# df07/mcp-raytracer

Hardware: AMD Instinct MI355X
Metric: Msamples/sec (w×h×spp/s) Cornell 800×800 spp=256 @1/2/4/8 GPU (higher is better)
Workload: dtype f64

## Files before the change

### include/rt_amd.h

```cpp
#ifndef RT_AMD_H
#define RT_AMD_H

#include <stddef.h>
#include <stdint.h>

#ifdef __cplusplus
extern "C" {
#endif

#define RT_AMD_VERSION 3

enum {
    RT_OK = 0,
    RT_ERR_INVALID = 1,
    RT_ERR_DEVICE = 2,
    RT_ERR_RENDER = 3
};

enum { RT_PRECISION_REF = 0, RT_PRECISION_FP32 = 1 };
enum { RT_TRAVERSAL_FAST = 0, RT_TRAVERSAL_REFERENCE = 1, RT_TRAVERSAL_BRUTE = 2, RT_TRAVERSAL_AUTO = 3 };

typedef struct rt_camera rt_camera;

typedef struct {
// ... 63 lines not shown
                            uint64_t* work_counters);

int rt_camera_export(const rt_camera* cam, void* nodes, void* prims, void* materials, void* lights,
                     int32_t* prim_object);

int rt_debug_world_hit(rt_camera* cam, int32_t traversal, int32_t n, const float* orig, const float* dir,
                       double* out);

int rt_debug_math(int32_t n, const uint32_t* u, double* out);

int rt_debug_fp64(int32_t n, const double* x, double* out);

int rt_debug_pass_plan(int64_t units, int64_t unit_slots, int64_t chunks_per_slot, int64_t rec_bytes_per_unit,
                       int64_t budget_bytes, int64_t* pass_units);

int rt_debug_rng(uint32_t seed, uint32_t pixel, uint32_t sample, int32_t n, uint32_t* out);

int rt_device_count(int32_t* count);

int rt_camera_kernel_times(rt_camera* cam, float* path_ms, float* accum_ms);

#define RT_STATS_WORDS 8
int rt_camera_stats_words(rt_camera* cam, uint64_t* dst, void* stream);

int rt_camera_adaptive_info(rt_camera* cam, int32_t* rounds, uint64_t* samples_rendered);

int rt_camera_pass_count(rt_camera* cam, int32_t* passes);

enum { RT_KERNEL_NONE = 0, RT_KERNEL_SEQUENTIAL = 1, RT_KERNEL_CHUNKED = 2, RT_KERNEL_POOL = 3 };
int rt_camera_last_kernel(rt_camera* cam, int32_t* kernel);
// ... 104 lines not shown
```

### mcp-raytracer_amd/csrc/rt_api.cpp

```cpp
#include <hip/hip_runtime.h>

#include <dlfcn.h>
#include <rccl/rccl.h>

#include <algorithm>
#include <cmath>
#include <cstddef>
#include <cstdio>
#include <cstdlib>
#include <cstring>
#include <exception>
#include <functional>
#include <memory>
#include <mutex>
#include <stdexcept>
#include <string>
#include <thread>
#include <type_traits>
#include <vector>

#include "../../include/rt_amd.h"
#include "denoise.hpp"
#include "json.hpp"
#include "launch.hpp"
#include "progressive.hpp"
#include "scene.hpp"

using namespace rt;

std::vector<uint8_t> rt_png_encode_device(const uint8_t* d_rgb, int32_t w, int32_t h, hipStream_t stream);

static_assert(ST_WORDS == RT_STATS_WORDS, "rt_camera_stats_words layout");

#ifndef RT_BUILD_ID
#define RT_BUILD_ID "unhashed"
#endif

namespace {

// ... 210 lines not shown
    DevCtx(const CamHost& h, int dev, int inst) : host(h), build(h.build), device(dev), instance(inst) {}
    DevCtx(const DevCtx&) = delete;
    DevCtx& operator=(const DevCtx&) = delete;

    uint4* d_blob = nullptr;
    int32_t lds_words = 0;
    int32_t lds_words2 = 0;
    int32_t off_prims = 0, off_mats = 0, off_lights = 0, off_nodes = 0, off_tprims = 0, off_tsph = 0, off_onbs = 0;
    int32_t off_tsph2 = -1;
    int32_t off_pre = 0, n_pre = 0, off_xrec = 0;
    int32_t n_onb = 0;
    int lds_max = 64 * 1024;
    std::vector<hipEvent_t> ev;
    int n_passes = 0;
    bool ev_accum = false;
    int last_kernel = RT_KERNEL_NONE;
    unsigned long long* d_stats = nullptr;
    unsigned long long* d_counters = nullptr;
    unsigned int* d_tile = nullptr;
    uint8_t* d_rgb = nullptr;
    float* d_rad = nullptr;
    int cus = 256;

    hipStream_t stream = nullptr;
    hipEvent_t ev_rendered = nullptr, ev_gather0 = nullptr, ev_gather1 = nullptr;
    uint8_t* d_slab = nullptr;
    float* d_rslab = nullptr;
    uint8_t* d_gather = nullptr;
    float* d_rgather = nullptr;
    size_t slab_cap = 0, rslab_cap = 0, gather_cap = 0, rgather_cap = 0;
    unsigned long long* h_words = nullptr;
    int h_words_cap = 0;

    ~DevCtx() {
// ... 32 lines not shown
        if (h_words_cap < n) {
            if (h_words) (void)hipHostFree(h_words);
            h_words = nullptr;
            h_words_cap = 0;
            hip_check(hipHostMalloc((void**)&h_words, (size_t)n * ST_WORDS * sizeof(unsigned long long), 0),
                      "hipHostMalloc");
            h_words_cap = n;
        }
    }

    void release() {
        if (!live) return;
        int prev = 0;
        (void)hipGetDevice(&prev);
        (void)hipSetDevice(device);
        for (void* p : {(void*)d_blob, (void*)d_stats, (void*)d_counters, (void*)d_tile, (void*)d_rgb, (void*)d_rad,
                        (void*)d_sbuf})
            if (p) (void)hipFree(p);
        d_blob = nullptr;
        d_stats = nullptr;
        d_counters = nullptr;
        d_tile = nullptr;
        d_rgb = nullptr;
        d_rad = nullptr;
        d_sbuf = nullptr;
        sbuf_cap = 0;
        free_adapt_buffers();
        prog_free();
        dn.free();
        if (d_prim_object) (void)hipFree(d_prim_object);
        d_prim_object = nullptr;
        for (hipEvent_t& e : dn_ev)
            if (e) (void)hipEventDestroy(e), e = nullptr;
// ... 143 lines not shown
        append(blob, build.tsph, &off_tsph);
        append(blob, build.prims, &off_prims);
        append(blob, exact_records(build.prims), &off_xrec);
        lds_words = (int32_t)(blob.size() / 16);
        append(blob, build.mats, &off_mats);
        append(blob, build.lights, &off_lights);
        const std::vector<RtOnb> onbs = planar_onbs(build.prims, &n_onb);
        append(blob, onbs, &off_onbs);
        lds_words2 = (int32_t)(blob.size() / 16);
        append(blob, build.nodes, &off_nodes);
        append(blob, prefilter_records(build.prims, &n_pre), &off_pre);
        off_tsph2 = -1;
        if (!build.tsph2.empty()) append(blob, build.tsph2, &off_tsph2);
        hip_check(hipMalloc(&d_blob, std::max<size_t>(blob.size(), 16)), "hipMalloc");
        if (!blob.empty()) hip_check(hipMemcpy(d_blob, blob.data(), blob.size(), hipMemcpyHostToDevice), "hipMemcpy");
        hip_check(hipMalloc(&d_stats, ST_WORDS * kStatStride * sizeof(unsigned long long)), "hipMalloc");
        hip_check(hipMalloc(&d_counters, kCounterWords * sizeof(unsigned long long)), "hipMalloc");
        hip_check(hipMalloc(&d_tile, 64), "hipMalloc");
        live = true;
        cus = device_cus(dev);
        int smem = 0;
        if (hipDeviceGetAttribute(&smem, hipDeviceAttributeMaxSharedMemoryPerBlock, dev) == hipSuccess && smem > 0)
            lds_max = smem;
    }

    void ensure_frame() {
        if (d_rgb) return;
        const size_t px = (size_t)build.cam.width * build.cam.height;
        hip_check(hipMalloc(&d_rgb, std::max<size_t>(px * 3, 1)), "hipMalloc");
        hip_check(hipMalloc(&d_rad, std::max<size_t>(px * 3, 1) * sizeof(float)), "hipMalloc");
    }

    hipEvent_t pass_event(int p, int k) {
        while ((int)ev.size() < 3 * (p + 1)) {
            hipEvent_t e = nullptr;
            hip_check(hipEventCreate(&e), "hipEventCreate");
            ev.push_back(e);
        }
        return ev[3 * p + k];
    }

    int effective_traversal(int trav) const { return host.effective_traversal(trav); }

    void times(float* path_ms, float* accum_ms) {
        *path_ms = 0.0f;
        *accum_ms = 0.0f;
        for (int p = 0; p < n_passes; ++p) {
            float a = 0.0f, b = 0.0f;
            hip_check(hipEventSynchronize(ev[3 * p + 1]), "hipEventSynchronize");
            hip_check(hipEventElapsedTime(&a, ev[3 * p], ev[3 * p + 1]), "hipEventElapsedTime");
            *path_ms += a;
            if (ev_accum) {
                hip_check(hipEventSynchronize(ev[3 * p + 2]), "hipEventSynchronize");
                hip_check(hipEventElapsedTime(&b, ev[3 * p + 1], ev[3 * p + 2]), "hipEventElapsedTime");
                *accum_ms += b;
            }
        }
    }

    DevScene dev_scene() const {
        DevScene S;
        const char* b = reinterpret_cast<const char*>(d_blob);
        S.tnodes = reinterpret_cast<const RtTNode*>(b);
        S.prims = reinterpret_cast<const RtPrim*>(b + off_prims);
        S.gprims = S.prims;
        S.gpre = reinterpret_cast<const RtPre*>(b + off_pre);
        S.n_pre = n_pre;
        S.xrec = reinterpret_cast<const RtExact*>(b + off_xrec);
        S.off_xrec = off_xrec;
// ... 20 lines not shown
        S.t4_stride = (int32_t)sizeof(RtT4Node);
        S.n_top = 0;
        S.top_lds = nullptr;
        S.nearfar = 0;
        S.troot = build.t4root;
        S.root_box = build.troot_box;
        S.cam = build.cam;
        S.mix_total = host.mix_total;
        S.light_w = host.light_w;
        return S;
    }

    void launch(const rt_region& region, int tile_group, int tile_groups, int prec, int trav, int count,
                uint8_t* rgb, float* rad, int32_t* pxs, int32_t* pxb, int packed, hipStream_t stream,
                int prog_len = 0) {
        const RtCamera& C = build.cam;
        if (tile_groups < 1 || tile_group < 0 || tile_group >= tile_groups)
            throw std::invalid_argument("tile_group must satisfy 0 <= tile_group < tile_groups");
        const int x0 = std::max(region.x, 0), y0 = std::max(region.y, 0);
        const int x1 = std::min(region.x + region.width, C.width);
        const int y1 = std::min(region.y + region.height, C.height);
        RtRegion reg{x0, y0, std::max(x1 - x0, 0), std::max(y1 - y0, 0), tile_group, tile_groups};
        const int tiles_x = (reg.width + kTile - 1) / kTile;
        const int tiles_y = (reg.height + kTile - 1) / kTile;
        const long total = (long)tiles_x * tiles_y;
        const long mine = total > tile_group ? (total - tile_group + tile_groups - 1) / tile_groups : 0;
        LaunchGeom g;
        g.tiles_x = std::max(tiles_x, 1);
        g.my_tiles = (int)mine;
        const long want = (mine + (kBlock / kWave) - 1) / (kBlock / kWave);
// ... 21 lines not shown
        if (g.lds_level == 0 && v.trav == TRAV_FAST && lds_scene_enabled() && env_flag("RT_AMD_TOP_CACHE", true)) {
            const size_t room = lds_cap > stack ? lds_cap - stack : 0;
            n_top = (int32_t)std::min<size_t>(build.t4nodes.size(), room / node_lds);
            g.lds_bytes = stack + (size_t)n_top * node_lds;
        }
        v.defer = v.trav == TRAV_FAST &&
                  env_flag("RT_AMD_DEFER", g.lds_level >= 1 && C.n_prims >= 100);
        if (g.lds_bytes + static_lds_bytes(count, false) > (size_t)lds_max)
            throw std::runtime_error("traversal stack exceeds the workgroup LDS (BVH too deep)");
        if (env_flag("RT_AMD_LAUNCH_LOG", false))
            std::fprintf(stderr,
                         "[rt launch] prims %d stack_depth %d trav %d lds_level %d lds %zu B (stack %zu, scene L1 %d / "
                         "L2 %d B) lds_max %d tiles %ld\n",
                         C.n_prims, C.stack_depth, v.trav, g.lds_level, g.lds_bytes, stack, lds_words * 16,
                         lds_words2 * 16, lds_max, mine);
        RenderOut out{rgb, rad, pxs, pxb, d_stats, d_counters, d_tile, packed ? 1 : 0};
        hip_check(launch_init_stats(d_stats, count ? d_counters : nullptr, d_tile, stream), "init_stats");
        n_passes = 0;
        last_kernel = RT_KERNEL_NONE;
        adapt_rounds = 0;
        adapt_rendered = 0;
        if (mine == 0) return;
        DevScene S = dev_scene();
        S.lds_stack_bytes = (int32_t)stack;
        S.lds_words = g.lds_level == 2 ? lds_words2 : lds_words;
        S.lds_node_pad = g.lds_level > 0 ? node_pad : 0;
        S.n_top = n_top;
        S.tsph2 = off_tsph2 >= 0 ? reinterpret_cast<const RtLeafSph*>(reinterpret_cast<const char*>(d_blob) + off_tsph2)
                                 : nullptr;
        if (g.lds_level == 0 && v.trav == TRAV_FAST && !S.tsph2 && C.n_prims > 0)
            throw std::runtime_error("fast traversal without leaf records");
        const bool chunked = env_flag("RT_AMD_CHUNKED", true);
        const bool rounds = C.adaptive && count != 1 && env_flag("RT_AMD_ADAPT_ROUNDS", true);
        if (prog_len <= 0 && (C.n_samples <= 0 || !chunked || (C.adaptive && !rounds))) {
            hip_check(hipEventRecord(pass_event(0, 0), stream), "hipEventRecord");
            hipError_t e = prec == PREC_FP32 ? launch_render_fp32(v, S, reg, out, g, nullptr, stream)
                                             : launch_render_ref(v, S, reg, out, g, nullptr, stream);
            hip_check(e, "pt_render_kernel launch");
            hip_check(hipEventRecord(pass_event(0, 1), stream), "hipEventRecord");
            n_passes = 1;
            ev_accum = false;
            last_kernel = RT_KERNEL_SEQUENTIAL;
            return;
        }
        SampleBuf sb{};

        S.lds_pool_off = (int32_t)((g.lds_bytes + 15) / 16 * 16);
        const bool pool_ok = !v.emit && (count == 0 || (RT_POOL_PROF && count == 2 && prec == PREC_REF)) && v.trav == TRAV_BRUTE && C.width < 65536 && C.height < 65536 &&
                 C.n_samples <= 65535 && C.depth <= 250 && build.mats.size() < (1u << 21) &&
// ... 46 lines not shown
            if (covered != nsamp) throw std::runtime_error("guided schedule: coverage");
            for (int p = 0; p < np; ++p) sb.rnch[p] = 1.0 / (double)sb.nch[p];
            sb.refill_min = std::min(env_int("RT_AMD_REFILL", 4), kWave);
            sb.min_ready = std::min(env_int("RT_AMD_READY", gtree ? 40 : 48), kWave);
        };
        int pass = 0;
        auto run_pass = [&](bool first) {
            const long group_slots = ((long)sb.slots + kWave - 1) / kWave * kWave;
            long items = 0;
            for (int p = 0; p < sb.n_phases; ++p) {
                sb.item_base[p] = (int32_t)items;
                items += group_slots * sb.nch[p];
            }
            if (items >= kItemCap) throw std::runtime_error("chunked pass too large");
            sb.n_items = (int32_t)items;
            if (!first) hip_check(hipMemsetAsync(d_tile, 0, 2 * sizeof(unsigned int), stream), "hipMemsetAsync");
            LaunchGeom gp = g;
            const int block = v.pool ? kBlockPool : kBlockChunk;
            gp.grid = (int)std::max<long>(1, std::min<long>(items / block + 1, (long)cus));
            DevScene Sp = S;
            if (v.pool) gp.lds_bytes = (size_t)S.lds_pool_off + pool_lds_bytes();
            hip_check(hipEventRecord(pass_event(pass, 0), stream), "hipEventRecord");
            hipError_t e = prec == PREC_FP32 ? launch_render_fp32(v, Sp, reg, out, gp, &sb, stream)
                                             : launch_render_ref(v, Sp, reg, out, gp, &sb, stream);
            hip_check(e, "pt_chunk_kernel launch");
            hip_check(hipEventRecord(pass_event(pass, 1), stream), "hipEventRecord");
        };
        if (prog_len > 0) {
            launch_progressive(S, reg, out, g, sb, schedule, run_pass, pass, stream, prog_len);
        } else if (rounds) {
            launch_adaptive_rounds(S, reg, out, g, mine, sb, schedule, run_pass, pass, stream);
        } else {
            sb.rec12 = C.mode != MODE_BOUNCES && !out.px_bounces && env_flag("RT_AMD_REC12", true);
            const size_t rec_per_tile = (size_t)kWave * (size_t)C.n_samples * (sb.rec12 ? 12 : sizeof(float4));
            schedule((double)mine * kWave, C.n_samples);
            const long pass_tiles = pass_units(mine, kWave, chunks_per_slot(sb), rec_per_tile, sbuf_budget());
            ensure_sbuf((size_t)pass_tiles * rec_per_tile);
            sb.rec = d_sbuf;
            for (long t0 = 0; t0 < mine; t0 += pass_tiles, ++pass) {
                const long nt = std::min(pass_tiles, mine - t0);
                sb.tile0 = (int32_t)t0;
                sb.slots = (int32_t)(nt * kWave);
                if (env_flag("RT_AMD_REC_SLOT_MAJOR", false)) {
                    sb.stride_s = 1;
                    sb.stride_slot = C.n_samples;
                } else {
                    sb.stride_s = sb.slots;
                    sb.stride_slot = 1;
                }
                run_pass(t0 == 0);
                hip_check(launch_accum(S, reg, out, g.tiles_x, sb, stream), "pt_accum_kernel launch");
                hip_check(hipEventRecord(pass_event(pass, 2), stream), "hipEventRecord");
            }
        }
        n_passes = pass;
        ev_accum = true;
        last_kernel = v.pool ? RT_KERNEL_POOL : RT_KERNEL_CHUNKED;
    }

    template <class Sched, class Pass>
    void launch_adaptive_rounds(DevScene& S, const RtRegion& reg, const RenderOut& out, const LaunchGeom& g, long mine,
                                SampleBuf& sb, Sched& schedule, Pass& run_pass, int& pass, hipStream_t stream) {
        const RtCamera& C = build.cam;
        const long slots_all = mine * kWave;
        ensure_adapt((size_t)slots_all);
        const double ab = C.a_batch;
        const int batch = (ab >= 1.0 && ab < 65536.0) ? (int)ab : std::max(1, std::min(C.n_samples, 16));
        int len = batch * std::max(1, (env_int("RT_AMD_ADAPT_FIRST", batch) + batch - 1) / batch);
// ... 138 lines not shown

    void prog_read(hipStream_t stream) {
        ProgSession& P = prog;
        unsigned long long wl[ST_WORDS * kStatStride];
        hip_check(hipMemcpyAsync(wl, d_stats, sizeof wl, hipMemcpyDeviceToHost, stream), "hipMemcpyAsync");
        hip_check(hipMemcpyAsync(P.h_count, P.d_count, 2 * sizeof(unsigned int), hipMemcpyDeviceToHost, stream),
                  "hipMemcpyAsync");
        hip_check(hipStreamSynchronize(stream), "hipStreamSynchronize");
        for (int k = 0; k < ST_WORDS; ++k) P.words[k] = wl[k * kStatStride];
        P.err |= P.words[ST_ERROR];
        P.words[ST_ERROR] = P.err;
        P.n_act = (long)P.h_count[0];
    }

    void prog_start(hipStream_t stream) {
        hip_check(launch_init_stats(d_stats, nullptr, d_tile, stream), "init_stats");
        prog_resolve(stream);
        prog_read(stream);
    }

    template <class Sched, class Pass>
    void launch_progressive(DevScene& S, const RtRegion& reg, const RenderOut& out, const LaunchGeom& g, SampleBuf& sb,
                            Sched& schedule, Pass& run_pass, int& pass, hipStream_t stream, int len) {
        ProgSession& P = prog;
        const long n_act = P.n_act;
        sb.s_base = P.done;
        sb.err_in_rec = 1;
        sb.rec12 = 0;
        sb.stride_slot = 1;
        sb.tile0 = 0;
        schedule((double)n_act, len);
        const size_t rec_per_slot = (size_t)len * sizeof(float4);
        const long pass_slots =
// ... 58 lines not shown
        free_adapt_buffers();
        hip_check(hipMalloc(&d_astate, slots * sizeof(AdaptPix)), "hipMalloc(adaptive state)");
        hip_check(hipMalloc(&d_act[0], slots * sizeof(int32_t)), "hipMalloc(active list)");
        hip_check(hipMalloc(&d_act[1], slots * sizeof(int32_t)), "hipMalloc(active list)");
        adapt_cap = slots;
    }
    void free_adapt_buffers() {
        for (void* p : {(void*)d_astate, (void*)d_act[0], (void*)d_act[1]})
            if (p) (void)hipFree(p);
        d_astate = nullptr;
        d_act[0] = d_act[1] = nullptr;
        adapt_cap = 0;
    }

    float4* d_sbuf = nullptr;
    size_t sbuf_cap = 0;
    void ensure_sbuf(size_t bytes) {
        if (bytes <= sbuf_cap) return;
        if (d_sbuf) (void)hipFree(d_sbuf);
        d_sbuf = nullptr;
        sbuf_cap = 0;
        hip_check(hipMalloc(&d_sbuf, bytes), "hipMalloc(sample buffer)");
        sbuf_cap = bytes;
    }
    static long chunks_per_slot(const SampleBuf& sb) {
        long n = 0;
        for (int p = 0; p < sb.n_phases; ++p) n += sb.nch[p];
        return n;
    }
    static size_t sbuf_budget() {
        const char* e = std::getenv("RT_AMD_SBUF_MB");
        const long mb = e ? std::atol(e) : 8192;
        return (size_t)std::max<long>(mb, 1) << 20;
    }

    void read_stats(rt_render_stats* st, uint64_t* counters, hipStream_t stream) {
        unsigned long long wl[ST_WORDS * kStatStride], w[ST_WORDS];
        hip_check(hipMemcpyAsync(wl, d_stats, sizeof wl, hipMemcpyDeviceToHost, stream), "hipMemcpyAsync");
// ... 199 lines not shown

    std::vector<std::exception_ptr> errs(n);
    auto work = [&](int g) {
        try {
            DevCtx& c = *cs[g];
            hip_check(hipSetDevice(c.device), "hipSetDevice");
            c.ensure_device();
            c.ensure_multi(slab_b, rslab_b, g == 0, n);
            if (g == 0) c.ensure_frame();
            c.launch(plan.region, g, n, cam->precision, cam->traversal, 0, c.d_slab, want_rad ? c.d_rslab : nullptr,
                     nullptr, nullptr, 1, c.stream);
            hip_check(hipMemcpy2DAsync(c.d_slab + plan.stats_offset, sizeof(unsigned long long), c.d_stats,
                                       kStatStride * sizeof(unsigned long long), sizeof(unsigned long long), ST_WORDS,
                                       hipMemcpyDeviceToDevice, c.stream),
                      "hipMemcpy2DAsync(stats)");
            hip_check(hipEventRecord(c.ev_rendered, c.stream), "hipEventRecord");
        } catch (...) {
            errs[g] = std::current_exception();
        }
    };
    std::vector<std::thread> th;
    for (int g = 1; g < n; ++g) th.emplace_back(work, g);
    work(0);
    for (auto& t : th) t.join();
    for (auto& e : errs)
        if (e) std::rethrow_exception(e);

    DevCtx& root = *cs[0];
    hip_check(hipSetDevice(root.device), "hipSetDevice");
    hip_check(hipEventRecord(root.ev_gather0, root.stream), "hipEventRecord");
// ... 518 lines not shown
        if (d_out) (void)hipFree(d_out);
        return set_error(RT_ERR_DEVICE, e.what());
    }
}

int rt_debug_pass_plan(int64_t units, int64_t unit_slots, int64_t chunks_per_slot, int64_t rec_bytes_per_unit,
                       int64_t budget_bytes, int64_t* pass_units_out) {
    if (units < 0 || unit_slots < 1 || chunks_per_slot < 1 || rec_bytes_per_unit < 1 || budget_bytes < 1 ||
        !pass_units_out)
        return set_error(RT_ERR_INVALID, "bad arguments");
    *pass_units_out = pass_units((long)units, (long)unit_slots, (long)chunks_per_slot, (size_t)rec_bytes_per_unit,
                                 (size_t)budget_bytes);
    return RT_OK;
}

int rt_debug_rng(uint32_t seed, uint32_t pixel, uint32_t sample, int32_t n, uint32_t* out) {
    if (n < 0 || (n > 0 && !out)) return set_error(RT_ERR_INVALID, "bad arguments");
    uint64_t s = splitmix64((((uint64_t)pixel << 32) | sample) ^ splitmix64(seed));
    for (int32_t k = 0; k < n; ++k) {
        const uint64_t old = s;
        s = old * 6364136223846793005ull + 1442695040888963407ull;
        const uint32_t xs = (uint32_t)(((old >> 18u) ^ old) >> 27u);
        const uint32_t rot = (uint32_t)(old >> 59u);
        out[k] = (xs >> rot) | (xs << ((32u - rot) & 31u));
    }
    return RT_OK;
}

int rt_camera_kernel_times(rt_camera* cam, float* path_ms, float* accum_ms) {
    if (!cam || !path_ms || !accum_ms) return set_error(RT_ERR_INVALID, "null argument");
// ... 5 lines not shown
        return RT_OK;
    } catch (const std::exception& e) {
        return set_error(RT_ERR_DEVICE, e.what());
    }
}

int rt_camera_stats_words(rt_camera* cam, uint64_t* dst, void* stream) {
    if (!cam || !dst) return set_error(RT_ERR_INVALID, "null argument");
    std::lock_guard<std::mutex> lock(cam->mu);
    try {
        DevCtx* c = cam->last;
        if (!c || !c->live || !c->d_stats) throw std::invalid_argument("rt_camera_stats_words: no render yet");
        hip_check(hipMemcpy2DAsync(dst, sizeof(uint64_t), c->d_stats, kStatStride * sizeof(unsigned long long),
                                   sizeof(uint64_t), ST_WORDS, hipMemcpyDeviceToDevice, (hipStream_t)stream),
                  "hipMemcpy2DAsync(stats)");
        return RT_OK;
    } catch (const std::invalid_argument& e) {
        return set_error(RT_ERR_INVALID, e.what());
    } catch (const std::exception& e) {
        return set_error(RT_ERR_DEVICE, e.what());
    }
}

int rt_camera_adaptive_info(rt_camera* cam, int32_t* rounds, uint64_t* samples_rendered) {
    if (!cam || !rounds || !samples_rendered) return set_error(RT_ERR_INVALID, "null argument");
    std::lock_guard<std::mutex> lock(cam->mu);
    *rounds = cam->last ? cam->last->adapt_rounds : 0;
    *samples_rendered = cam->last ? cam->last->adapt_rendered : 0;
    return RT_OK;
}
// ... 527 lines not shown
```

### mcp-raytracer_amd/raytracer_amd/_build.py

```python
from __future__ import annotations

import hashlib
import os
import shutil
import subprocess
from concurrent.futures import ThreadPoolExecutor
from pathlib import Path

PKG_DIR = Path(__file__).resolve().parent
CSRC = PKG_DIR.parent / "csrc"
INCLUDE = PKG_DIR.parent.parent / "include"
LIB_DIR = PKG_DIR / "lib"
LIB_PATH = LIB_DIR / "librt_amd.so"
OBJ_DIR = PKG_DIR.parent / "build"

ARCH = "gfx950"

_COMMON = ["-std=c++17", "-O3", "-fPIC", "-Wall", "-Wno-unused-function", "-Wno-unused-variable",
           f"-I{CSRC}", f"-I{INCLUDE}"]

_KERNEL_FLAGS = ["-fno-slp-vectorize", "-mllvm", "-disable-machine-licm"]
_UNITS = [
    ("pt_ref.hip", ["-ffp-contract=off", *_KERNEL_FLAGS], True),
    ("pt_fp32.hip", ["-ffp-contract=fast", *_KERNEL_FLAGS], True),
    ("progressive.hip", ["-ffp-contract=off", *_KERNEL_FLAGS], True),
    ("denoise.hip", ["-ffp-contract=off", *_KERNEL_FLAGS], True),
    ("frame.hip", [], True),
    ("png.hip", [], True),
    ("rt_api.cpp", ["-ffp-contract=off", "-x", "hip"], True),
    ("scene.cpp", ["-ffp-contract=off"], False),
    ("image.cpp", [], False),
]
_HEADERS = ["json.hpp", "rt_math.hpp", "scene.hpp", "pt_kernel.hpp", "launch.hpp", "progressive.hpp", "denoise.hpp",
            "png_deflate.hpp"]
_LIBS = ["-lz"]


def source_hash(defines=(), flags=()) -> str:
    h = hashlib.sha256()
    for name in [u[0] for u in _UNITS] + _HEADERS:
        h.update(name.encode() + b"\0" + (CSRC / name).read_bytes())
    h.update((INCLUDE / "rt_amd.h").read_bytes())
    h.update(repr((ARCH, _COMMON[:3], [(u[0], u[1]) for u in _UNITS], _LIBS, list(defines), list(flags))).encode())
    return h.hexdigest()[:16]


def id_path(lib_path: Path) -> Path:
    return lib_path.with_name(lib_path.name + ".id")

# ... 76 lines not shown
```

### mcp-raytracer_amd/raytracer_amd/_lib.py

```python
from __future__ import annotations

import ctypes as C
import json
import os
from pathlib import Path

from ._build import LIB_PATH, id_path, source_hash

HEADER = Path(__file__).resolve().parents[2] / "include" / "rt_amd.h"

RT_OK, RT_ERR_INVALID, RT_ERR_DEVICE, RT_ERR_RENDER = 0, 1, 2, 3
PRECISION = {"ref": 0, "fp32": 1}
TRAVERSAL = {"fast": 0, "reference": 1, "brute": 2, "auto": 3}

CT_NAMES = ["node", "sphere", "quad", "plane", "material", "light_quad", "light_sphere",
            "bounces", "diffuse", "samples", "rays", "exact", "exact_wave", "cand0", "cand2", "exact2"]
PR_NAMES = ["newpath", "rr", "hit", "miss", "hitrec", "scatter", "sample", "pdf", "acc", "tile", "node", "leaf",
            "wnode", "wleaf", "loop", "trips"]
COUNTER_WORDS = 64
STATS_WORDS = 8


class RtRegion(C.Structure):
    _fields_ = [("x", C.c_int32), ("y", C.c_int32), ("width", C.c_int32), ("height", C.c_int32)]
# ... 54 lines not shown
                "samples_done": self.samples_done, "samples": self.samples, "steps": self.steps,
                "done": bool(self.done), "precision": "fp32" if self.precision == 1 else "ref", "seed": self.seed,
                "active_pixels": self.active_pixels, "state_bytes": self.state_bytes,
                "build_id": self.build_id.decode()}


class RtDenoiseOptions(C.Structure):
    _fields_ = [("levels", C.c_int32), ("sigma_color", C.c_float), ("sigma_plane", C.c_float)]


class RtDenoiseVarOptions(C.Structure):
    _fields_ = [("levels", C.c_int32), ("sigma_variance", C.c_float), ("sigma_plane", C.c_float)]


DENOISE_MAX_LEVELS = 8


class RtError(RuntimeError):

    def __init__(self, code: int, message: str):
        super().__init__(message)
        self.code = code


_SIGS = {
    "rt_version": (C.c_int, []),
    "rt_last_error": (C.c_char_p, []),
    "rt_free": (None, [C.c_void_p]),
    "rt_generate_scene_data": (C.c_int, [C.c_char_p, C.c_char_p, C.POINTER(C.c_void_p)]),
    "rt_camera_create": (C.c_int, [C.c_char_p, C.c_char_p, C.POINTER(C.c_void_p)]),
    "rt_camera_destroy": (None, [C.c_void_p]),
    "rt_camera_get_info": (C.c_int, [C.c_void_p, C.POINTER(RtCameraInfo)]),
    "rt_camera_set_precision": (C.c_int, [C.c_void_p, C.c_int32]),
    "rt_camera_render_region": (C.c_int, [C.c_void_p, C.POINTER(RtRegion), C.c_void_p, C.c_void_p,
                                          C.POINTER(RtRenderStats)]),
    "rt_camera_render": (C.c_int, [C.c_void_p, C.c_void_p, C.c_void_p, C.POINTER(RtRenderStats)]),
    "rt_camera_render_device": (C.c_int, [C.c_void_p, C.POINTER(RtLaunch), C.POINTER(RtRenderStats),
                                          C.POINTER(C.c_uint64)]),
    "rt_camera_export": (C.c_int, [C.c_void_p, C.c_void_p, C.c_void_p, C.c_void_p, C.c_void_p,
                                   C.c_void_p]),
    "rt_debug_world_hit": (C.c_int, [C.c_void_p, C.c_int32, C.c_int32, C.c_void_p, C.c_void_p, C.c_void_p]),
    "rt_debug_pass_plan": (C.c_int, [C.c_int64, C.c_int64, C.c_int64, C.c_int64, C.c_int64,
                                     C.POINTER(C.c_int64)]),
    "rt_debug_rng": (C.c_int, [C.c_uint32, C.c_uint32, C.c_uint32, C.c_int32, C.c_void_p]),
    "rt_debug_math": (C.c_int, [C.c_int32, C.c_void_p, C.c_void_p]),
    "rt_debug_fp64": (C.c_int, [C.c_int32, C.c_void_p, C.c_void_p]),
    "rt_device_count": (C.c_int, [C.POINTER(C.c_int32)]),
    "rt_camera_kernel_times": (C.c_int, [C.c_void_p, C.POINTER(C.c_float), C.POINTER(C.c_float)]),
    "rt_camera_adaptive_info": (C.c_int, [C.c_void_p, C.POINTER(C.c_int32), C.POINTER(C.c_uint64)]),
    "rt_camera_stats_words": (C.c_int, [C.c_void_p, C.c_void_p, C.c_void_p]),
    "rt_camera_pass_count": (C.c_int, [C.c_void_p, C.POINTER(C.c_int32)]),
    "rt_camera_last_kernel": (C.c_int, [C.c_void_p, C.POINTER(C.c_int32)]),
    "rt_camera_release_device": (C.c_int, [C.c_void_p]),
    "rt_build_id": (C.c_char_p, []),
    "rt_tiles_unpack": (C.c_int, [C.c_void_p, C.c_int32, C.c_int32, C.POINTER(RtRegion), C.c_int32, C.c_int32,
                                  C.c_int32, C.c_int32, C.c_void_p, C.c_void_p]),
    "rt_encode_png": (C.c_int, [C.c_void_p, C.c_int32, C.c_int32, C.c_int32, C.POINTER(C.c_void_p),
                                C.POINTER(C.c_size_t)]),
# ... 85 lines not shown

def to_json(obj) -> bytes:
    return json.dumps(obj, allow_nan=True, separators=(",", ":")).encode()


def multi_plan(region, width: int, height: int, n_devices: int) -> dict:
    p = RtMultiPlan()
    reg = RtRegion(*[int(v) for v in region])
    check(load().rt_multi_plan_region(C.byref(reg), int(width), int(height), int(n_devices), C.byref(p)))
    return {"region": (p.region.x, p.region.y, p.region.width, p.region.height), "n_devices": p.n_devices,
            "slab_tiles": p.slab_tiles, "tiles": p.tiles, "slab_bytes_rgb": p.slab_bytes_rgb,
            "slab_bytes_radiance": p.slab_bytes_radiance, "stats_offset": p.stats_offset,
            "group_tiles": list(p.group_tiles)[:p.n_devices]}


def progressive_blob_info(blob: bytes) -> dict:
    info = RtProgressiveInfo()
    blob = bytes(blob)
    check(load().rt_progressive_blob_info(blob, len(blob), C.byref(info)))
    return info.as_dict()


def progressive_blob_variance(blob: bytes):
    import numpy as np
    blob = bytes(blob)
    info = progressive_blob_info(blob)
    var = np.zeros((info["height"], info["width"]), np.float32)
    check(load().rt_progressive_blob_variance(blob, len(blob), var.ctypes.data))
    return var

# ... 6 lines not shown
```

### mcp-raytracer_amd/raytracer_amd/camera.py

```python
from __future__ import annotations

import ctypes as C
import math
from dataclasses import dataclass, field
from typing import Iterable, Optional, Sequence

from . import _lib

RENDER_MODES = ("default", "bounces", "samples")


def _mm(total=0.0, mn=math.inf, mx=0.0, avg=0.0):
    return {"total": total, "min": mn, "max": mx, "avg": avg}


@dataclass
class RenderStats:

    pixels: float = 0
    samples: dict = field(default_factory=_mm)
    bounces: dict = field(default_factory=_mm)

    @classmethod
    def _from_c(cls, s: _lib.RtRenderStats) -> "RenderStats":
# ... 258 lines not shown
        return float(a.value), float(b.value)

    def stats_words(self, dst_ptr: int, stream=None) -> None:
        _lib.check(self._lib.rt_camera_stats_words(self._h, C.c_void_p(dst_ptr), C.c_void_p(stream)))

    def adaptive_info(self):
        r, n = C.c_int32(), C.c_uint64()
        _lib.check(self._lib.rt_camera_adaptive_info(self._h, C.byref(r), C.byref(n)))
        return int(r.value), int(n.value)

    def pass_count(self) -> int:
        n = C.c_int32()
        _lib.check(self._lib.rt_camera_pass_count(self._h, C.byref(n)))
        return int(n.value)

    KERNELS = ("none", "sequential", "chunked", "pool")

    def last_kernel(self) -> str:
        n = C.c_int32()
        _lib.check(self._lib.rt_camera_last_kernel(self._h, C.byref(n)))
        return self.KERNELS[int(n.value)]

    def progressive(self, region=None) -> "ProgressiveRender":
        reg = None if region is None else _region(region)
        _lib.check(self._lib.rt_camera_progressive_begin(self._h, C.byref(reg) if reg is not None else None))
        return ProgressiveRender(self)

    def resume(self, blob: bytes) -> "ProgressiveRender":
        blob = bytes(blob)
        _lib.check(self._lib.rt_camera_progressive_restore(self._h, blob, len(blob)))
# ... 204 lines not shown
```

Before: 12120.

## Pipeline path-trace and accumulation passes with double-buffered sample records

Adds a second sample-record buffer and a second stats/counter/tile block, and runs the chunked path-tracing kernel on a separate non-blocking stream. The accumulation kernel stays on the caller stream and the two are ordered through a small event plan, so pass N's accumulate can overlap pass N+1's path kernel and a new launch can start while the previous one's accumulate is still running. This targets serialisation between passes and between back-to-back launches. In exchange it costs extra device memory for the second record buffer, adds event bookkeeping on every launch, and risks ordering bugs around stats reads, which is why block_read hooks are added.

```diff
diff --git a/include/rt_amd.h b/include/rt_amd.h
--- a/include/rt_amd.h
+++ b/include/rt_amd.h
@@ -101,6 +101,31 @@
 int rt_debug_pass_plan(int64_t units, int64_t unit_slots, int64_t chunks_per_slot, int64_t rec_bytes_per_unit,
                        int64_t budget_bytes, int64_t* pass_units);
 
+enum {
+    RT_PIPE_PATH0 = 1, RT_PIPE_PATH1 = 2, RT_PIPE_ACC0 = 4, RT_PIPE_ACC1 = 8, RT_PIPE_BLK0 = 16, RT_PIPE_BLK1 = 32
+};
+typedef struct {
+    int32_t have_second;
+    int32_t last_buf;
+    int32_t last_blk;
+    int32_t recorded;
+    int32_t tail;
+} rt_pipe_state;
+typedef struct {
+    int32_t pipelined;
+    int32_t buf, blk;
+    int32_t init_block;
+    int32_t alloc_second;
+    int32_t internal_waits;
+    int32_t internal_records;
+    int32_t caller_waits;
+    int32_t caller_records;
+} rt_pipe_pass;
+int rt_debug_pipeline_plan(rt_pipe_state* state, int32_t pipelined, int32_t passes, int32_t first_buffer_idle,
+                           rt_pipe_pass* out);
+
+int rt_camera_record_bytes(rt_camera* cam, int64_t* first, int64_t* second);
+
 int rt_debug_rng(uint32_t seed, uint32_t pixel, uint32_t sample, int32_t n, uint32_t* out);
 
 int rt_device_count(int32_t* count);
diff --git a/mcp-raytracer_amd/csrc/pipeline.hpp b/mcp-raytracer_amd/csrc/pipeline.hpp
--- /dev/null
+++ b/mcp-raytracer_amd/csrc/pipeline.hpp
@@ -0,0 +1,60 @@
+#pragma once
+
+#include <cstdint>
+
+#include "../../include/rt_amd.h"
+
+namespace rt {
+
+constexpr int32_t pipe_path_bit(int buf) { return buf ? RT_PIPE_PATH1 : RT_PIPE_PATH0; }
+constexpr int32_t pipe_acc_bit(int buf) { return buf ? RT_PIPE_ACC1 : RT_PIPE_ACC0; }
+constexpr int32_t pipe_blk_bit(int blk) { return blk ? RT_PIPE_BLK1 : RT_PIPE_BLK0; }
+constexpr int kPipeEvents = 6;
+
+inline rt_pipe_pass pipe_plan_pass(rt_pipe_state& s, bool pipelined, bool first, bool buf0_idle) {
+    rt_pipe_pass p{};
+    p.pipelined = pipelined ? 1 : 0;
+    p.init_block = first ? 1 : 0;
+    if (!pipelined) {
+        p.buf = 0;
+        p.blk = s.last_blk;
+        if (first) {
+            p.caller_waits = s.tail;
+            s.tail = 0;
+        }
+        s.last_buf = 0;
+        return p;
+    }
+    p.blk = first && (s.recorded & (RT_PIPE_BLK0 | RT_PIPE_BLK1)) ? 1 - s.last_blk : s.last_blk;
+    if (s.have_second) {
+        p.buf = 1 - s.last_buf;
+    } else if ((s.recorded & RT_PIPE_ACC0) && !(first && buf0_idle)) {
+        p.buf = 1;
+        p.alloc_second = 1;
+        s.have_second = 1;
+    } else {
+        p.buf = 0;
+    }
+    p.internal_waits = s.recorded & (pipe_acc_bit(p.buf) | (first ? pipe_blk_bit(p.blk) : 0));
+    p.internal_records = pipe_path_bit(p.buf);
+    p.caller_waits = pipe_path_bit(p.buf);
+    p.caller_records = pipe_acc_bit(p.buf);
+    s.recorded |= p.internal_records | p.caller_records;
+    s.tail = pipe_path_bit(p.buf);
+    s.last_buf = p.buf;
+    s.last_blk = p.blk;
+    return p;
+}
+
+inline int32_t pipe_plan_end(rt_pipe_state& s, bool pipelined) {
+    const int32_t r = pipe_blk_bit(s.last_blk) | (pipelined ? 0 : RT_PIPE_ACC0);
+    s.recorded |= r;
+    return r;
+}
+
+inline void pipe_plan_launch(rt_pipe_state& s, bool pipelined, int passes, bool buf0_idle, rt_pipe_pass* out) {
+    for (int p = 0; p < passes; ++p) out[p] = pipe_plan_pass(s, pipelined, p == 0, p == 0 && buf0_idle);
+    out[passes - 1].caller_records |= pipe_plan_end(s, pipelined);
+}
+
+}
diff --git a/mcp-raytracer_amd/csrc/rt_api.cpp b/mcp-raytracer_amd/csrc/rt_api.cpp
--- a/mcp-raytracer_amd/csrc/rt_api.cpp
+++ b/mcp-raytracer_amd/csrc/rt_api.cpp
@@ -23,6 +23,7 @@
 #include "denoise.hpp"
 #include "json.hpp"
 #include "launch.hpp"
+#include "pipeline.hpp"
 #include "progressive.hpp"
 #include "scene.hpp"
 
@@ -263,10 +264,18 @@
     std::vector<hipEvent_t> ev;
     int n_passes = 0;
     bool ev_accum = false;
+    bool ev_split = false;
     int last_kernel = RT_KERNEL_NONE;
     unsigned long long* d_stats = nullptr;
     unsigned long long* d_counters = nullptr;
     unsigned int* d_tile = nullptr;
+    unsigned long long* blk_stats[2] = {nullptr, nullptr};
+    unsigned long long* blk_counters[2] = {nullptr, nullptr};
+    unsigned int* blk_tile[2] = {nullptr, nullptr};
+    hipStream_t pipe_stream = nullptr;
+    rt_pipe_state pipe{};
+    hipEvent_t pipe_ev[kPipeEvents] = {};
+    bool launch_pipelined = false;
     uint8_t* d_rgb = nullptr;
     float* d_rad = nullptr;
     int cus = 256;
@@ -329,9 +338,26 @@
         int prev = 0;
         (void)hipGetDevice(&prev);
         (void)hipSetDevice(device);
-        for (void* p : {(void*)d_blob, (void*)d_stats, (void*)d_counters, (void*)d_tile, (void*)d_rgb, (void*)d_rad,
-                        (void*)d_sbuf})
+        if (pipe_stream) {
+            (void)hipStreamSynchronize(pipe_stream);
+            (void)hipStreamDestroy(pipe_stream);
+            pipe_stream = nullptr;
+        }
+        for (hipEvent_t& e : pipe_ev)
+            if (e) (void)hipEventDestroy(e), e = nullptr;
+        pipe = rt_pipe_state{};
+        launch_pipelined = false;
+        for (void* p : {(void*)d_blob, (void*)blk_stats[0], (void*)blk_stats[1], (void*)blk_counters[0],
+                        (void*)blk_counters[1], (void*)blk_tile[0], (void*)blk_tile[1], (void*)d_rgb, (void*)d_rad,
+                        (void*)d_sbuf, (void*)d_sbuf2})
             if (p) (void)hipFree(p);
+        for (int b = 0; b < 2; ++b) {
+            blk_stats[b] = nullptr;
+            blk_counters[b] = nullptr;
+            blk_tile[b] = nullptr;
+        }
+        d_sbuf2 = nullptr;
+        sbuf2_cap = 0;
         d_blob = nullptr;
         d_stats = nullptr;
         d_counters = nullptr;
@@ -505,9 +531,12 @@
         if (!build.tsph2.empty()) append(blob, build.tsph2, &off_tsph2);
         hip_check(hipMalloc(&d_blob, std::max<size_t>(blob.size(), 16)), "hipMalloc");
         if (!blob.empty()) hip_check(hipMemcpy(d_blob, blob.data(), blob.size(), hipMemcpyHostToDevice), "hipMemcpy");
-        hip_check(hipMalloc(&d_stats, ST_WORDS * kStatStride * sizeof(unsigned long long)), "hipMalloc");
-        hip_check(hipMalloc(&d_counters, kCounterWords * sizeof(unsigned long long)), "hipMalloc");
-        hip_check(hipMalloc(&d_tile, 64), "hipMalloc");
+        for (int b = 0; b < 2; ++b) {
+            hip_check(hipMalloc(&blk_stats[b], ST_WORDS * kStatStride * sizeof(unsigned long long)), "hipMalloc");
+            hip_check(hipMalloc(&blk_counters[b], kCounterWords * sizeof(unsigned long long)), "hipMalloc");
+            hip_check(hipMalloc(&blk_tile[b], 64), "hipMalloc");
+        }
+        select_block(0);
         live = true;
         cus = device_cus(dev);
         int smem = 0;
@@ -523,12 +552,56 @@
     }
 
     hipEvent_t pass_event(int p, int k) {
-        while ((int)ev.size() < 3 * (p + 1)) {
+        while ((int)ev.size() < 4 * (p + 1)) {
             hipEvent_t e = nullptr;
             hip_check(hipEventCreate(&e), "hipEventCreate");
             ev.push_back(e);
         }
-        return ev[3 * p + k];
+        return ev[4 * p + k];
+    }
+
+    void select_block(int b) {
+        d_stats = blk_stats[b];
+        d_counters = blk_counters[b];
+        d_tile = blk_tile[b];
+    }
+    template <class F>
+    void pipe_events(int32_t mask, F&& f) {
+        for (int k = 0; k < kPipeEvents; ++k) {
+            if (!(mask >> k & 1)) continue;
+            if (!pipe_ev[k]) hip_check(hipEventCreateWithFlags(&pipe_ev[k], hipEventDisableTiming), "hipEventCreate");
+            f(pipe_ev[k]);
+        }
+    }
+    void pipe_wait(hipStream_t s, int32_t mask) {
+        pipe_events(mask, [&](hipEvent_t e) { hip_check(hipStreamWaitEvent(s, e, 0), "hipStreamWaitEvent"); });
+    }
+    void pipe_record(hipStream_t s, int32_t mask) {
+        pipe_events(mask, [&](hipEvent_t e) { hip_check(hipEventRecord(e, s), "hipEventRecord"); });
+    }
+    bool pipe_buf0_idle() {
+        if (!(pipe.recorded & RT_PIPE_ACC0) || !pipe_ev[2]) return true;
+        const hipError_t e = hipEventQuery(pipe_ev[2]);
+        if (e == hipErrorNotReady) return false;
+        hip_check(e, "hipEventQuery");
+        return true;
+    }
+    void serial_begin(hipStream_t stream) {
+        const rt_pipe_pass pp = pipe_plan_pass(pipe, false, true, false);
+        launch_pipelined = false;
+        select_block(pp.blk);
+        pipe_wait(stream, pp.caller_waits);
+    }
+    void serial_end(hipStream_t stream) { pipe_record(stream, pipe_plan_end(pipe, false)); }
+    void block_read(hipStream_t stream) { pipe_record(stream, pipe_blk_bit(pipe.last_blk)); }
+    void pipe_abort(hipStream_t stream) {
+        (void)stream;
+        (void)hipDeviceSynchronize();
+        rt_pipe_state s{};
+        s.have_second = d_sbuf2 ? 1 : 0;
+        pipe = s;
+        launch_pipelined = false;
+        if (blk_stats[0]) select_block(0);
     }
 
     int effective_traversal(int trav) const { return host.effective_traversal(trav); }
@@ -538,12 +611,12 @@
         *accum_ms = 0.0f;
         for (int p = 0; p < n_passes; ++p) {
             float a = 0.0f, b = 0.0f;
-            hip_check(hipEventSynchronize(ev[3 * p + 1]), "hipEventSynchronize");
-            hip_check(hipEventElapsedTime(&a, ev[3 * p], ev[3 * p + 1]), "hipEventElapsedTime");
+            hip_check(hipEventSynchronize(ev[4 * p + 1]), "hipEventSynchronize");
+            hip_check(hipEventElapsedTime(&a, ev[4 * p], ev[4 * p + 1]), "hipEventElapsedTime");
             *path_ms += a;
             if (ev_accum) {
-                hip_check(hipEventSynchronize(ev[3 * p + 2]), "hipEventSynchronize");
-                hip_check(hipEventElapsedTime(&b, ev[3 * p + 1], ev[3 * p + 2]), "hipEventElapsedTime");
+                hip_check(hipEventSynchronize(ev[4 * p + 2]), "hipEventSynchronize");
+                hip_check(hipEventElapsedTime(&b, ev[4 * p + (ev_split ? 3 : 1)], ev[4 * p + 2]), "hipEventElapsedTime");
                 *accum_ms += b;
             }
         }
@@ -594,6 +667,18 @@
     void launch(const rt_region& region, int tile_group, int tile_groups, int prec, int trav, int count,
                 uint8_t* rgb, float* rad, int32_t* pxs, int32_t* pxb, int packed, hipStream_t stream,
                 int prog_len = 0) {
+        try {
+            launch_impl(region, tile_group, tile_groups, prec, trav, count, rgb, rad, pxs, pxb, packed, stream, prog_len);
+            pipe_record(stream, pipe_plan_end(pipe, launch_pipelined));
+        } catch (...) {
+            pipe_abort(stream);
+            throw;
+        }
+    }
+
+    void launch_impl(const rt_region& region, int tile_group, int tile_groups, int prec, int trav, int count,
+                     uint8_t* rgb, float* rad, int32_t* pxs, int32_t* pxb, int packed, hipStream_t stream,
+                     int prog_len) {
         const RtCamera& C = build.cam;
         if (tile_groups < 1 || tile_group < 0 || tile_group >= tile_groups)
             throw std::invalid_argument("tile_group must satisfy 0 <= tile_group < tile_groups");
@@ -645,9 +730,24 @@
                          "L2 %d B) lds_max %d tiles %ld\n",
                          C.n_prims, C.stack_depth, v.trav, g.lds_level, g.lds_bytes, stack, lds_words * 16,
                          lds_words2 * 16, lds_max, mine);
+        const bool chunked = env_flag("RT_AMD_CHUNKED", true);
+        const bool rounds = C.adaptive && count != 1 && env_flag("RT_AMD_ADAPT_ROUNDS", true);
+        const bool sequential = prog_len <= 0 && (C.n_samples <= 0 || !chunked || (C.adaptive && !rounds));
+        launch_pipelined = mine > 0 && prog_len <= 0 && !sequential && !rounds && env_flag("RT_AMD_PIPELINE", true);
+        hipStream_t path_stream = stream;
+        rt_pipe_pass pp0 = pipe_plan_pass(pipe, launch_pipelined, true, launch_pipelined && pipe_buf0_idle());
+        select_block(pp0.blk);
+        if (launch_pipelined) {
+            if (!pipe_stream) hip_check(hipStreamCreateWithFlags(&pipe_stream, hipStreamNonBlocking), "hipStreamCreate");
+            path_stream = pipe_stream;
+            pipe_wait(path_stream, pp0.internal_waits);
+        } else {
+            pipe_wait(stream, pp0.caller_waits);
+        }
         RenderOut out{rgb, rad, pxs, pxb, d_stats, d_counters, d_tile, packed ? 1 : 0};
-        hip_check(launch_init_stats(d_stats, count ? d_counters : nullptr, d_tile, stream), "init_stats");
+        hip_check(launch_init_stats(d_stats, count ? d_counters : nullptr, d_tile, path_stream), "init_stats");
         n_passes = 0;
+        ev_split = false;
         last_kernel = RT_KERNEL_NONE;
         adapt_rounds = 0;
         adapt_rendered = 0;
@@ -661,9 +761,7 @@
                                  : nullptr;
         if (g.lds_level == 0 && v.trav == TRAV_FAST && !S.tsph2 && C.n_prims > 0)
             throw std::runtime_error("fast traversal without leaf records");
-        const bool chunked = env_flag("RT_AMD_CHUNKED", true);
-        const bool rounds = C.adaptive && count != 1 && env_flag("RT_AMD_ADAPT_ROUNDS", true);
-        if (prog_len <= 0 && (C.n_samples <= 0 || !chunked || (C.adaptive && !rounds))) {
+        if (sequential) {
             hip_check(hipEventRecord(pass_event(0, 0), stream), "hipEventRecord");
             hipError_t e = prec == PREC_FP32 ? launch_render_fp32(v, S, reg, out, g, nullptr, stream)
                                              : launch_render_ref(v, S, reg, out, g, nullptr, stream);
@@ -740,17 +838,17 @@
             }
             if (items >= kItemCap) throw std::runtime_error("chunked pass too large");
             sb.n_items = (int32_t)items;
-            if (!first) hip_check(hipMemsetAsync(d_tile, 0, 2 * sizeof(unsigned int), stream), "hipMemsetAsync");
+            if (!first) hip_check(hipMemsetAsync(d_tile, 0, 2 * sizeof(unsigned int), path_stream), "hipMemsetAsync");
             LaunchGeom gp = g;
             const int block = v.pool ? kBlockPool : kBlockChunk;
             gp.grid = (int)std::max<long>(1, std::min<long>(items / block + 1, (long)cus));
             DevScene Sp = S;
             if (v.pool) gp.lds_bytes = (size_t)S.lds_pool_off + pool_lds_bytes();
-            hip_check(hipEventRecord(pass_event(pass, 0), stream), "hipEventRecord");
-            hipError_t e = prec == PREC_FP32 ? launch_render_fp32(v, Sp, reg, out, gp, &sb, stream)
-                                             : launch_render_ref(v, Sp, reg, out, gp, &sb, stream);
+            hip_check(hipEventRecord(pass_event(pass, 0), path_stream), "hipEventRecord");
+            hipError_t e = prec == PREC_FP32 ? launch_render_fp32(v, Sp, reg, out, gp, &sb, path_stream)
+                                             : launch_render_ref(v, Sp, reg, out, gp, &sb, path_stream);
             hip_check(e, "pt_chunk_kernel launch");
-            hip_check(hipEventRecord(pass_event(pass, 1), stream), "hipEventRecord");
+            hip_check(hipEventRecord(pass_event(pass, 1), path_stream), "hipEventRecord");
         };
         if (prog_len > 0) {
             launch_progressive(S, reg, out, g, sb, schedule, run_pass, pass, stream, prog_len);
@@ -761,9 +859,11 @@
             const size_t rec_per_tile = (size_t)kWave * (size_t)C.n_samples * (sb.rec12 ? 12 : sizeof(float4));
             schedule((double)mine * kWave, C.n_samples);
             const long pass_tiles = pass_units(mine, kWave, chunks_per_slot(sb), rec_per_tile, sbuf_budget());
-            ensure_sbuf((size_t)pass_tiles * rec_per_tile);
-            sb.rec = d_sbuf;
             for (long t0 = 0; t0 < mine; t0 += pass_tiles, ++pass) {
+                const rt_pipe_pass pp = t0 == 0 ? pp0 : pipe_plan_pass(pipe, launch_pipelined, false, false);
+                ensure_sbuf((size_t)pass_tiles * rec_per_tile, pp.buf);
+                sb.rec = pp.buf ? d_sbuf2 : d_sbuf;
+                if (t0 > 0) pipe_wait(path_stream, pp.internal_waits);
                 const long nt = std::min(pass_tiles, mine - t0);
                 sb.tile0 = (int32_t)t0;
                 sb.slots = (int32_t)(nt * kWave);
@@ -775,9 +875,16 @@
                     sb.stride_slot = 1;
                 }
                 run_pass(t0 == 0);
+                pipe_record(path_stream, pp.internal_records);
+                if (launch_pipelined) {
+                    pipe_wait(stream, pp.caller_waits);
+                    hip_check(hipEventRecord(pass_event(pass, 3), stream), "hipEventRecord");
+                }
                 hip_check(launch_accum(S, reg, out, g.tiles_x, sb, stream), "pt_accum_kernel launch");
                 hip_check(hipEventRecord(pass_event(pass, 2), stream), "hipEventRecord");
+                pipe_record(stream, pp.caller_records);
             }
+            ev_split = launch_pipelined;
         }
         n_passes = pass;
         ev_accum = true;
@@ -946,9 +1053,11 @@
     }
 
     void prog_start(hipStream_t stream) {
+        serial_begin(stream);
         hip_check(launch_init_stats(d_stats, nullptr, d_tile, stream), "init_stats");
         prog_resolve(stream);
         prog_read(stream);
+        serial_end(stream);
     }
 
     template <class Sched, class Pass>
@@ -1037,14 +1146,17 @@
     }
 
     float4* d_sbuf = nullptr;
-    size_t sbuf_cap = 0;
-    void ensure_sbuf(size_t bytes) {
-        if (bytes <= sbuf_cap) return;
-        if (d_sbuf) (void)hipFree(d_sbuf);
-        d_sbuf = nullptr;
-        sbuf_cap = 0;
-        hip_check(hipMalloc(&d_sbuf, bytes), "hipMalloc(sample buffer)");
-        sbuf_cap = bytes;
+    float4* d_sbuf2 = nullptr;
+    size_t sbuf_cap = 0, sbuf2_cap = 0;
+    void ensure_sbuf(size_t bytes, int which = 0) {
+        float4*& buf = which ? d_sbuf2 : d_sbuf;
+        size_t& cap = which ? sbuf2_cap : sbuf_cap;
+        if (bytes <= cap) return;
+        if (buf) (void)hipFree(buf);
+        buf = nullptr;
+        cap = 0;
+        hip_check(hipMalloc(&buf, bytes), "hipMalloc(sample buffer)");
+        cap = bytes;
     }
     static long chunks_per_slot(const SampleBuf& sb) {
         long n = 0;
@@ -1274,6 +1386,7 @@
                                        kStatStride * sizeof(unsigned long long), sizeof(unsigned long long), ST_WORDS,
                                        hipMemcpyDeviceToDevice, c.stream),
                       "hipMemcpy2DAsync(stats)");
+            c.block_read(c.stream);
             hip_check(hipEventRecord(c.ev_rendered, c.stream), "hipEventRecord");
         } catch (...) {
             errs[g] = std::current_exception();
@@ -1822,6 +1935,26 @@
     return RT_OK;
 }
 
+int rt_debug_pipeline_plan(rt_pipe_state* state, int32_t pipelined, int32_t passes, int32_t first_buffer_idle,
+                           rt_pipe_pass* out) {
+    if (!state || !out || passes < 1) return set_error(RT_ERR_INVALID, "rt_debug_pipeline_plan: bad arguments");
+    pipe_plan_launch(*state, pipelined != 0, passes, first_buffer_idle != 0, out);
+    return RT_OK;
+}
+
+int rt_camera_record_bytes(rt_camera* cam, int64_t* first, int64_t* second) {
+    if (!cam || !first || !second) return set_error(RT_ERR_INVALID, "null argument");
+    std::lock_guard<std::mutex> lock(cam->mu);
+    try {
+        DevCtx& c = cam->current();
+        *first = (int64_t)c.sbuf_cap;
+        *second = (int64_t)c.sbuf2_cap;
+        return RT_OK;
+    } catch (const std::exception& e) {
+        return set_error(RT_ERR_DEVICE, e.what());
+    }
+}
+
 int rt_debug_rng(uint32_t seed, uint32_t pixel, uint32_t sample, int32_t n, uint32_t* out) {
     if (n < 0 || (n > 0 && !out)) return set_error(RT_ERR_INVALID, "bad arguments");
     uint64_t s = splitmix64((((uint64_t)pixel << 32) | sample) ^ splitmix64(seed));
@@ -1857,6 +1990,7 @@
         hip_check(hipMemcpy2DAsync(dst, sizeof(uint64_t), c->d_stats, kStatStride * sizeof(unsigned long long),
                                    sizeof(uint64_t), ST_WORDS, hipMemcpyDeviceToDevice, (hipStream_t)stream),
                   "hipMemcpy2DAsync(stats)");
+        c->block_read((hipStream_t)stream);
         return RT_OK;
     } catch (const std::invalid_argument& e) {
         return set_error(RT_ERR_INVALID, e.what());
diff --git a/mcp-raytracer_amd/raytracer_amd/_build.py b/mcp-raytracer_amd/raytracer_amd/_build.py
--- a/mcp-raytracer_amd/raytracer_amd/_build.py
+++ b/mcp-raytracer_amd/raytracer_amd/_build.py
@@ -32,7 +32,7 @@
     ("image.cpp", [], False),
 ]
 _HEADERS = ["json.hpp", "rt_math.hpp", "scene.hpp", "pt_kernel.hpp", "launch.hpp", "progressive.hpp", "denoise.hpp",
-            "png_deflate.hpp"]
+            "png_deflate.hpp", "pipeline.hpp"]
 _LIBS = ["-lz"]
 
 
diff --git a/mcp-raytracer_amd/raytracer_amd/_lib.py b/mcp-raytracer_amd/raytracer_amd/_lib.py
--- a/mcp-raytracer_amd/raytracer_amd/_lib.py
+++ b/mcp-raytracer_amd/raytracer_amd/_lib.py
@@ -92,6 +92,24 @@
 
 
 DENOISE_MAX_LEVELS = 8
+
+PIPE_PATH = (1, 2)
+PIPE_ACC = (4, 8)
+PIPE_BLK = (16, 32)
+
+
+class RtPipeState(C.Structure):
+    _fields_ = [("have_second", C.c_int32), ("last_buf", C.c_int32), ("last_blk", C.c_int32),
+                ("recorded", C.c_int32), ("tail", C.c_int32)]
+
+
+class RtPipePass(C.Structure):
+    _fields_ = [("pipelined", C.c_int32), ("buf", C.c_int32), ("blk", C.c_int32), ("init_block", C.c_int32),
+                ("alloc_second", C.c_int32), ("internal_waits", C.c_int32), ("internal_records", C.c_int32),
+                ("caller_waits", C.c_int32), ("caller_records", C.c_int32)]
+
+    def as_dict(self) -> dict:
+        return {name: int(getattr(self, name)) for name, _ in self._fields_}
 
 
 class RtError(RuntimeError):
@@ -120,6 +138,9 @@
     "rt_debug_world_hit": (C.c_int, [C.c_void_p, C.c_int32, C.c_int32, C.c_void_p, C.c_void_p, C.c_void_p]),
     "rt_debug_pass_plan": (C.c_int, [C.c_int64, C.c_int64, C.c_int64, C.c_int64, C.c_int64,
                                      C.POINTER(C.c_int64)]),
+    "rt_debug_pipeline_plan": (C.c_int, [C.POINTER(RtPipeState), C.c_int32, C.c_int32, C.c_int32,
+                                         C.POINTER(RtPipePass)]),
+    "rt_camera_record_bytes": (C.c_int, [C.c_void_p, C.POINTER(C.c_int64), C.POINTER(C.c_int64)]),
     "rt_debug_rng": (C.c_int, [C.c_uint32, C.c_uint32, C.c_uint32, C.c_int32, C.c_void_p]),
     "rt_debug_math": (C.c_int, [C.c_int32, C.c_void_p, C.c_void_p]),
     "rt_debug_fp64": (C.c_int, [C.c_int32, C.c_void_p, C.c_void_p]),
@@ -235,6 +256,13 @@
             "group_tiles": list(p.group_tiles)[:p.n_devices]}
 
 
+def pipeline_plan(state: RtPipeState, pipelined: bool, passes: int, first_buffer_idle: bool) -> list:
+    out = (RtPipePass * int(passes))()
+    check(load().rt_debug_pipeline_plan(C.byref(state), int(bool(pipelined)), int(passes),
+                                        int(bool(first_buffer_idle)), out))
+    return [p.as_dict() for p in out]
+
+
 def progressive_blob_info(blob: bytes) -> dict:
     info = RtProgressiveInfo()
     blob = bytes(blob)
diff --git a/mcp-raytracer_amd/raytracer_amd/camera.py b/mcp-raytracer_amd/raytracer_amd/camera.py
--- a/mcp-raytracer_amd/raytracer_amd/camera.py
+++ b/mcp-raytracer_amd/raytracer_amd/camera.py
@@ -296,6 +296,11 @@
         _lib.check(self._lib.rt_camera_pass_count(self._h, C.byref(n)))
         return int(n.value)
 
+    def record_bytes(self):
+        a, b = C.c_int64(), C.c_int64()
+        _lib.check(self._lib.rt_camera_record_bytes(self._h, C.byref(a), C.byref(b)))
+        return int(a.value), int(b.value)
+
     KERNELS = ("none", "sequential", "chunked", "pool")
 
     def last_kernel(self) -> str:
```

Measured after the change: 12220, median of 6. Within noise of the previous version (+0.8%).
